# LordLiang/DrawingSpinUp

Measured on AMD Instinct MI355X. Metric: drawings/sec end-to-end (512x512, 6 views, 24 frames), higher is better.
Workload: dtype f16 (diffusion) / f16 table + f32 MLP (NSR) / f32 (stage-1 deformable convolutions, IS-Net, contour) / f32 with bf16 x 3 products (stage-2 convolutions; the reference: cuDNN TF32)

## Files before the change

### drawingspinup_amd/csrc/adamw_dev.h

```cpp
#pragma once
#include "common.h"
#include <hip/hip_fp16.h>

struct dsu_table_adamw_args {
  float4 *p, *g, *m, *v;
  __half2* img;
  int64_t n4;
  float lr, beta1, beta2, eps, wd, bc1, bc2_sqrt;
};

__device__ __forceinline__ void dsu_table_adamw_range(const dsu_table_adamw_args& a, int64_t first,
                                                      int64_t stride) {
  const float step_size = a.lr / a.bc1;
  const float omb1 = (float)(1.0 - (double)a.beta1), omb2 = (float)(1.0 - (double)a.beta2);
  for (int64_t i = first; i < a.n4; i += stride) {
    float4 P = a.p[i], G = a.g[i], M = a.m[i], V = a.v[i];
    float* pp = &P.x; float* gg = &G.x; float* mm = &M.x; float* vv = &V.x;
#pragma unroll
    for (int k = 0; k < 4; ++k) {
      float x = pp[k];
      x -= a.lr * a.wd * x;
      const float mk = mm[k] + (gg[k] - mm[k]) * omb1;
      const float vk = a.beta2 * vv[k] + omb2 * gg[k] * gg[k];
      const float denom = sqrtf(vk) / a.bc2_sqrt + a.eps;
      x -= step_size * mk / denom;
      pp[k] = x; mm[k] = mk; vv[k] = vk;
    }
    a.p[i] = P; a.m[i] = M; a.v[i] = V;
    a.g[i] = make_float4(0.0f, 0.0f, 0.0f, 0.0f);
    a.img[2 * i] = __floats2half2_rn(P.x, P.y);
    a.img[2 * i + 1] = __floats2half2_rn(P.z, P.w);
  }
}
```

### drawingspinup_amd/csrc/nsr_driver.hip

```cpp
#include "common.h"
#include "adamw_dev.h"

#include <math.h>
#include <string.h>

#include <mutex>
#include <vector>

namespace {

constexpr int N_GEO = 64 * 23 + 64 + 13 * 64 + 13;
constexpr int N_TEX = 64 * 16 + 64 + 64 * 64 + 64 + 3 * 64 + 3;
constexpr int N_SMALL = (64 * 23 + 64 + 64) + (13 * 64 + 13 + 13) + N_TEX + 1;

__device__ __forceinline__ uint4 philox(uint4 c, uint2 k) {
#pragma unroll
  for (int i = 0; i < 10; ++i) {
    const uint32_t hi0 = __umulhi(0xD2511F53u, c.x), lo0 = 0xD2511F53u * c.x;
    const uint32_t hi1 = __umulhi(0xCD9E8D57u, c.z), lo1 = 0xCD9E8D57u * c.z;
    c = make_uint4(hi1 ^ c.y ^ k.x, lo1, hi0 ^ c.w ^ k.y, lo0);
    k.x += 0x9E3779B9u;
    k.y += 0xBB67AE85u;
  }
  return c;
}
__device__ __forceinline__ float u01(uint32_t x) { return (float)(x >> 8) * (1.0f / 16777216.0f); }

__global__ __launch_bounds__(256) void nsr_draw_kernel(uint64_t seed, int64_t step, int32_t n_rays,
                                                       int32_t V, int32_t H, int32_t W,
                                                       int64_t* __restrict__ index,
                                                       int64_t* __restrict__ px,
                                                       int64_t* __restrict__ py,
                                                       float* __restrict__ jitter, int32_t n_random,
                                                       float* __restrict__ pts_random,
                                                       float* __restrict__ perturb) {
  const int i = blockIdx.x * blockDim.x + threadIdx.x;
  const uint2 key = make_uint2((uint32_t)seed, (uint32_t)(seed >> 32));
  const uint32_t s0 = (uint32_t)step, s1 = (uint32_t)((uint64_t)step >> 32);
  if (i < n_rays) {
    const uint4 r = philox(make_uint4((uint32_t)i, 0u, s0, s1), key);
    index[i] = (int64_t)(r.x % (uint32_t)V);
    px[i] = (int64_t)(r.y % (uint32_t)W);
    py[i] = (int64_t)(r.z % (uint32_t)H);
    jitter[i] = u01(r.w);
  }
  if (i < n_random) {
    const uint4 a = philox(make_uint4((uint32_t)i, 1u, s0, s1), key);
    const uint4 b = philox(make_uint4((uint32_t)i, 2u, s0, s1), key);
    pts_random[3 * i] = u01(a.x) * 2.0f - 1.0f;
    pts_random[3 * i + 1] = u01(a.y) * 2.0f - 1.0f;
    pts_random[3 * i + 2] = u01(a.z) * 2.0f - 1.0f;
    const float u1 = 1.0f - u01(b.x), u2 = u01(b.y), u3 = 1.0f - u01(b.z), u4 = u01(b.w);
    const float r1 = sqrtf(-2.0f * logf(u1)), r2 = sqrtf(-2.0f * logf(u3));
    perturb[3 * i] = r1 * cosf(6.28318530717958648f * u2);
    perturb[3 * i + 1] = r1 * sinf(6.28318530717958648f * u2);
    perturb[3 * i + 2] = r2 * cosf(6.28318530717958648f * u4);
  }
}

struct SmallArgs {
  float *w0_v, *w0_g, *b0, *w1_v, *w1_g, *b1;
  float* tex[6];
  float* variance;
  float* g_geo;
  float* g_tex;
  float* d_inv;
  float *m, *v;
  float *w0_eff, *w1_eff, *inv_s;
  float* zero_terms;
  const float* terms;
  float* terms_out;
  float lr_geo, lr_tex, lr_var, beta1, beta2, eps, wd, bc1, bc2_sqrt;
  int32_t update;
};

__device__ __forceinline__ void adamw_elem(float& x, float g, float& m, float& v, float lr,
                                           const SmallArgs& a) {
  const float omb1 = (float)(1.0 - (double)a.beta1), omb2 = (float)(1.0 - (double)a.beta2);
  x -= lr * a.wd * x;
  m = m + (g - m) * omb1;
  v = a.beta2 * v + omb2 * g * g;
  const float denom = sqrtf(v) / a.bc2_sqrt + a.eps;
  x -= (lr / a.bc1) * m / denom;
}

__global__ __launch_bounds__(1024) void small_update_kernel(SmallArgs a, dsu_table_adamw_args ta) {
  if (blockIdx.x > 0) {
    dsu_table_adamw_range(ta, (int64_t)(blockIdx.x - 1) * 1024 + threadIdx.x,
                          (int64_t)(gridDim.x - 1) * 1024);
    return;
  }
  __shared__ float s_g[N_GEO];
  __shared__ float s_v0[64 * 23], s_v1[13 * 64];
  __shared__ float s_gain[77], s_norm[77], s_dot[77];
  const int t = threadIdx.x;
  for (int i = t; i < 64 * 23; i += 1024) s_v0[i] = a.w0_v[i];
  for (int i = t; i < 13 * 64; i += 1024) s_v1[i] = a.w1_v[i];
  if (t < 77) s_gain[t] = t < 64 ? a.w0_g[t] : a.w1_g[t - 64];
  if (a.update)
    for (int i = t; i < N_GEO; i += 1024) s_g[i] = a.g_geo[i];
  __syncthreads();
  if (a.update) {
    if (t < 77) {
      const bool l0 = t < 64;
      const int r = l0 ? t : t - 64, cols = l0 ? 23 : 64;
      const float* vrow = (l0 ? s_v0 : s_v1) + r * cols;
      const float* grow = (l0 ? s_g : s_g + 64 * 23 + 64) + r * cols;
      float nn = 0.0f, dot = 0.0f;
      for (int c = 0; c < cols; ++c) {
        nn += vrow[c] * vrow[c];
        dot += grow[c] * vrow[c];
      }
      s_norm[t] = sqrtf(nn);
      s_dot[t] = dot;
    }
    __syncthreads();
    int off = 0;
    for (int i = t; i < 64 * 23; i += 1024) {
      const int r = i / 23;
      const float nrm = s_norm[r];
      const float g = (s_gain[r] / nrm) * (s_g[i] - s_v0[i] * s_dot[r] / (nrm * nrm));
      float x = s_v0[i], m = a.m[off + i], v = a.v[off + i];
      adamw_elem(x, g, m, v, a.lr_geo, a);
      a.w0_v[i] = x; a.m[off + i] = m; a.v[off + i] = v;
      s_v0[i] = x;
    }
    off += 64 * 23;
    float new_gain = 0.0f;
    if (t < 64) {
      float x = s_gain[t], m = a.m[off + t], v = a.v[off + t];
      adamw_elem(x, s_dot[t] / s_norm[t], m, v, a.lr_geo, a);
      a.w0_g[t] = x; a.m[off + t] = m; a.v[off + t] = v;
      new_gain = x;
    }
    off += 64;
    if (t < 64) {
      float x = a.b0[t], m = a.m[off + t], v = a.v[off + t];
      adamw_elem(x, s_g[64 * 23 + t], m, v, a.lr_geo, a);
      a.b0[t] = x; a.m[off + t] = m; a.v[off + t] = v;
    }
    off += 64;
    for (int i = t; i < 13 * 64; i += 1024) {
      const int r = i / 64;
      const float nrm = s_norm[64 + r];
      const float g = (s_gain[64 + r] / nrm) *
                      (s_g[64 * 23 + 64 + i] - s_v1[i] * s_dot[64 + r] / (nrm * nrm));
      float x = s_v1[i], m = a.m[off + i], v = a.v[off + i];
      adamw_elem(x, g, m, v, a.lr_geo, a);
      a.w1_v[i] = x; a.m[off + i] = m; a.v[off + i] = v;
      s_v1[i] = x;
    }
    off += 13 * 64;
    float new_gain1 = 0.0f;
    if (t < 13) {
      float x = s_gain[64 + t], m = a.m[off + t], v = a.v[off + t];
      adamw_elem(x, s_dot[64 + t] / s_norm[64 + t], m, v, a.lr_geo, a);
      a.w1_g[t] = x; a.m[off + t] = m; a.v[off + t] = v;
      new_gain1 = x;
    }
    off += 13;
    if (t < 13) {
      float x = a.b1[t], m = a.m[off + t], v = a.v[off + t];
      adamw_elem(x, s_g[64 * 23 + 64 + 13 * 64 + t], m, v, a.lr_geo, a);
      a.b1[t] = x; a.m[off + t] = m; a.v[off + t] = v;
    }
    off += 13;
    const int tn[6] = {64 * 16, 64, 64 * 64, 64, 3 * 64, 3};
    int go = 0;
    for (int k = 0; k < 6; ++k) {
      float* p = a.tex[k];
      for (int i = t; i < tn[k]; i += 1024) {
        float x = p[i], m = a.m[off + i], v = a.v[off + i];
        adamw_elem(x, a.g_tex[go + i], m, v, a.lr_tex, a);
        p[i] = x; a.m[off + i] = m; a.v[off + i] = v;
      }
      off += tn[k];
      go += tn[k];
    }
    if (t == 1023) {
      float x = a.variance[0], m = a.m[off], v = a.v[off];
      const float g = a.d_inv[0] * expf(x * 10.0f) * 10.0f;
      adamw_elem(x, g, m, v, a.lr_var, a);
      a.variance[0] = x; a.m[off] = m; a.v[off] = v;
      a.inv_s[0] = expf(x * 10.0f);
      a.d_inv[0] = 0.0f;
    }
    if (t < 3) a.zero_terms[t] = 0.0f;
    if (t >= 8 && t < 16 && a.terms_out) a.terms_out[t - 8] = a.terms[t - 8];
    __syncthreads();
    if (t < 64) s_gain[t] = new_gain;
    if (t < 13) s_gain[64 + t] = new_gain1;
    for (int i = t; i < N_GEO; i += 1024) a.g_geo[i] = 0.0f;
    for (int i = t; i < N_TEX; i += 1024) a.g_tex[i] = 0.0f;
    __syncthreads();
  } else if (t == 1023) {
    a.inv_s[0] = expf(a.variance[0] * 10.0f);
  }
  if (t < 77) {
    const bool l0 = t < 64;
    const int r = l0 ? t : t - 64, cols = l0 ? 23 : 64;
    const float* vrow = (l0 ? s_v0 : s_v1) + r * cols;
    float nn = 0.0f;
    for (int c = 0; c < cols; ++c) nn += vrow[c] * vrow[c];
    s_norm[t] = s_gain[t] / sqrtf(nn);
  }
  __syncthreads();
  for (int i = t; i < 64 * 23; i += 1024) a.w0_eff[i] = s_v0[i] * s_norm[i / 23];
  for (int i = t; i < 13 * 64; i += 1024) a.w1_eff[i] = s_v1[i] * s_norm[64 + i / 64];
}

struct Carve {
  char* base;
  int64_t off = 0;
  template <typename T>
  T* take(int64_t count) {
    off = (off + 255) / 256 * 256;
    T* p = base ? reinterpret_cast<T*>(base + off) : nullptr;
    off += count * (int64_t)sizeof(T);
    return p;
  }
};

struct Prefetch {
  int64_t *index, *px, *py;
  float *jitter, *rays, *rgb, *normal, *mask, *cosines, *vw, *tmin, *tmax;
  int32_t *counts, *offsets, *stats;
  float *rays_o, *rays_d;
  float *pts_random, *perturb;
  float *points, *t_starts, *t_ends, *sorted;
  int32_t* perm;
  void* sort_ws;
};

struct Layout {
  Prefetch pf[3];
  float *scratch_ts, *scratch_te;
  float *a_sdf, *a_grad, *a_feat;
  void* enc_cache;
  float *normal, *rgb, *alpha, *w, *comp, *d_comp, *terms;
  float *d_sdf_all, *d_grad_all, *d_feat_all, *d_normal, *d_rgb;
  void *tex_ws, *sdf_ws;
  int32_t* tex_map;
  uint32_t* tex_mask;
  float *g_geo, *g_tex, *d_inv;
  float *w0_eff, *w1_eff, *inv_s, *adam_m, *adam_v;
  int64_t tex_ws_bytes, sdf_ws_bytes, sort_ws_bytes, enc_cache_bytes, total;
};

int32_t march_row_capacity(float radius, float step) {
  const double diag = sqrt(3.0 * (2.0 * radius) * (2.0 * radius));
  return (int32_t)(diag / step) + 8;
}

int carve(const dsu_nsr_driver_cfg& c, char* base, Layout& L) {
  Carve k{base};
  const int64_t R = c.cap_rays, N = c.cap_points, nr = c.n_random, rows = N + 2 * nr;
  const int32_t rowcap = march_row_capacity(c.radius, c.render_step_size);
  L.sort_ws_bytes = c.sort_bits ? dsu_spatial_sort_workspace_bytes(rows, c.sort_bits) : 0;
  L.tex_ws_bytes = dsu_texture_bwd_workspace_bytes(N);
  L.sdf_ws_bytes = dsu_sdf_fd_bwd_workspace_bytes(&c.grid, rows);
  L.enc_cache_bytes = dsu_sdf_fd_enc_cache_bytes(rows, c.grid.n_levels);
  if (L.sort_ws_bytes < 0 || L.tex_ws_bytes < 0 || L.sdf_ws_bytes < 0 || L.enc_cache_bytes < 0)
    return DSU_EINVAL;
  for (int p = 0; p < 3; ++p) {
    Prefetch& f = L.pf[p];
    f.index = k.take<int64_t>(R); f.px = k.take<int64_t>(R); f.py = k.take<int64_t>(R);
    f.jitter = k.take<float>(R); f.rays = k.take<float>(R * 6); f.rgb = k.take<float>(R * 4);
    f.normal = k.take<float>(R * 3); f.mask = k.take<float>(R); f.cosines = k.take<float>(R);
    f.vw = k.take<float>(R); f.tmin = k.take<float>(R); f.tmax = k.take<float>(R);
    f.counts = k.take<int32_t>(R); f.offsets = k.take<int32_t>(R); f.stats = k.take<int32_t>(4);
    f.rays_o = k.take<float>(R * 3); f.rays_d = k.take<float>(R * 3);
    f.pts_random = k.take<float>(nr * 3); f.perturb = k.take<float>(nr * 3);
    f.points = k.take<float>(rows * 3); f.t_starts = k.take<float>(N); f.t_ends = k.take<float>(N);
    f.sorted = k.take<float>(rows * 3); f.perm = k.take<int32_t>(rows);
    f.sort_ws = k.take<char>(L.sort_ws_bytes > 4 ? L.sort_ws_bytes : 4);
  }
  L.scratch_ts = k.take<float>(R * (int64_t)rowcap);
  L.scratch_te = k.take<float>(R * (int64_t)rowcap);
  L.a_sdf = k.take<float>(rows); L.a_grad = k.take<float>(rows * 3); L.a_feat = k.take<float>(rows * 13);
  L.enc_cache = k.take<char>(L.enc_cache_bytes);
  L.normal = k.take<float>(N * 3); L.rgb = k.take<float>(N * 3);
  L.alpha = k.take<float>(N); L.w = k.take<float>(N);
  L.comp = k.take<float>(R * 8); L.d_comp = k.take<float>(R * 8); L.terms = k.take<float>(16);
  L.d_sdf_all = k.take<float>(rows); L.d_grad_all = k.take<float>(rows * 3);
  L.d_feat_all = k.take<float>(rows * 13);
  L.d_normal = k.take<float>(N * 3); L.d_rgb = k.take<float>(N * 3);
  L.tex_ws = k.take<char>(L.tex_ws_bytes > 4 ? L.tex_ws_bytes : 4);
  L.sdf_ws = k.take<char>(L.sdf_ws_bytes > 4 ? L.sdf_ws_bytes : 4);
  L.tex_map = k.take<int32_t>(dsu_texture_partial_map(nullptr));
  L.tex_mask = k.take<uint32_t>(N * 2);
  L.g_geo = k.take<float>(N_GEO + N_TEX + 1);
// ... 102 lines not shown
    DSU_HIP(hipMemcpy2DAsync(f.rays_d, 3 * sizeof(float), a.inj_rays + 3, 6 * sizeof(float),
                             3 * sizeof(float), n, hipMemcpyDeviceToDevice, s));
  } else {
    DSU_TRY(dsu_ortho_ray_batch_split(index, px, py, n_rays, c.c2w, c.origins, c.directions, c.images,
                                      c.image_channels, c.normals, c.masks, c.view_weights, c.H, c.W,
                                      f.rays, f.rgb, f.normal, f.mask, f.cosines, f.vw, f.rays_o,
                                      f.rays_d, s));
  }
  DSU_TRY(dsu_ray_aabb(f.rays_o, f.rays_d, n_rays, d->aabb, a.randomized ? jitter : nullptr,
                       c.render_step_size, f.tmin, f.tmax, s));
  DSU_TRY(dsu_ray_march_scratch(f.rays_o, f.rays_d, f.tmin, f.tmax, n_rays, d->aabb, a.occ_binary,
                                a.occ_binary ? a.occ_res : 0, c.render_step_size, d->rowcap,
                                f.counts, d->L.scratch_ts, d->L.scratch_te, s));
  return DSU_OK;
}

int enqueue_pack(dsu_nsr_driver* d, int p, int32_t n_rays, const dsu_nsr_step_args& a,
                 bool injected, hipStream_t s) {
  const dsu_nsr_driver_cfg& c = d->cfg;
  Prefetch& f = d->L.pf[p];
  const float* pts_random = (injected && a.inj_pts_random) ? a.inj_pts_random : f.pts_random;
  const float* perturb = (injected && a.inj_perturb) ? a.inj_perturb : f.perturb;
  DSU_TRY(dsu_ray_offsets(f.counts, n_rays, f.offsets, f.stats, s));
  DSU_TRY(dsu_ray_compact_points_cap(d->L.scratch_ts, d->L.scratch_te, d->rowcap, f.offsets,
                                     f.counts, n_rays, f.rays_o, f.rays_d, f.t_starts, f.t_ends,
                                     f.points, c.cap_points, s));
  DSU_TRY(dsu_points_tail(f.points, (int64_t)c.cap_points + 2 * c.n_random, f.stats, pts_random,
                          perturb, c.n_random, 1e-2f, s));
  if (c.sort_bits)
    DSU_TRY(dsu_spatial_sort_dev(f.points, (int64_t)c.cap_points + 2 * c.n_random, f.stats,
                                 2 * c.n_random, c.radius, c.sort_bits, f.perm, f.sorted,
                                 f.sort_ws, d->L.sort_ws_bytes, s));
  DSU_HIP(hipMemcpyAsync(d->host_stats + 2 * p, f.stats, 2 * sizeof(int32_t),
                         hipMemcpyDeviceToHost, s));
  return DSU_OK;
}

int enqueue_samples(dsu_nsr_driver* d, int p, int64_t step, int32_t n_rays,
                    const dsu_nsr_step_args& a, bool injected, hipStream_t s) {
  DSU_TRY(enqueue_march(d, p, step, n_rays, a, injected, s));
  return enqueue_pack(d, p, n_rays, a, injected, s);
}

int mark(dsu_nsr_driver* d, int family, hipStream_t s) {
  if (!d->timing) return DSU_OK;
  hipEvent_t e;
  DSU_HIP(hipEventCreate(&e));
  DSU_HIP(hipEventRecord(e, s));
  d->ev[family].push_back(e);
  return DSU_OK;
}

int launch_small_update(dsu_nsr_driver* d, const dsu_nsr_step_args* a, int update, hipStream_t s) {
  const dsu_nsr_driver_cfg& c = d->cfg;
  SmallArgs sa;
  sa.w0_v = c.w0_v; sa.w0_g = c.w0_g; sa.b0 = c.b0; sa.w1_v = c.w1_v; sa.w1_g = c.w1_g; sa.b1 = c.b1;
  for (int k = 0; k < 6; ++k) sa.tex[k] = c.tex[k];
  sa.variance = c.variance;
  sa.g_geo = d->L.g_geo; sa.g_tex = d->L.g_tex; sa.d_inv = d->L.d_inv;
  sa.m = d->L.adam_m; sa.v = d->L.adam_v;
  sa.w0_eff = d->L.w0_eff; sa.w1_eff = d->L.w1_eff; sa.inv_s = d->L.inv_s;
  sa.zero_terms = d->L.terms + 8 * (int)((a->step + 1) & 1) + 4;
  sa.terms = d->L.terms + 8 * (int)(a->step & 1);
  sa.terms_out = update ? a->terms_out : nullptr;
  sa.beta1 = c.beta1; sa.beta2 = c.beta2; sa.eps = c.adam_eps; sa.wd = c.weight_decay;
  sa.update = update;
  sa.lr_geo = sa.lr_tex = sa.lr_var = 0.0f;
  sa.bc1 = sa.bc2_sqrt = 1.0f;
  if (update) {
    sa.lr_geo = a->lr_geometry; sa.lr_tex = a->lr_texture; sa.lr_var = a->lr_variance;
    sa.bc1 = (float)(1.0 - pow((double)c.beta1, (double)a->adam_step));
    sa.bc2_sqrt = (float)sqrt(1.0 - pow((double)c.beta2, (double)a->adam_step));
  }
  dsu_table_adamw_args ta{};
  int table_blocks = 0;
  if (update && a->table_p) {
    if (a->table_n < 0 || (a->table_n & 3) || !a->table_grad || !a->table_m || !a->table_v ||
        !a->table_img || !(a->table_bc1 > 0.0f) || !(a->table_bc2_sqrt > 0.0f))
      return DSU_EINVAL;
    ta = dsu_table_adamw_args{(float4*)a->table_p, (float4*)a->table_grad, (float4*)a->table_m,
                              (float4*)a->table_v, (__half2*)const_cast<void*>(a->table_img),
                              a->table_n / 4, a->table_lr, c.beta1, c.beta2, a->table_eps,
                              a->table_wd, a->table_bc1, a->table_bc2_sqrt};
    table_blocks = (int)((ta.n4 + 1023) / 1024 < 512 ? (ta.n4 + 1023) / 1024 : 512);
  }
  small_update_kernel<<<dim3(1 + table_blocks), dim3(1024), 0, s>>>(sa, ta);
  DSU_CHECK_LAUNCH();
  return DSU_OK;
}

}

extern "C" {

int dsu_nsr_draws(uint64_t seed, int64_t step, int32_t n_rays, int32_t V, int32_t H, int32_t W,
                  int64_t* index, int64_t* x, int64_t* y, float* jitter, int32_t n_random,
                  float* pts_random, float* perturb, void* stream) {
  if (n_rays < 0 || n_random < 0 || V < 1 || H < 1 || W < 1 ||
      (n_rays && (!index || !x || !y || !jitter)) || (n_random && (!pts_random || !perturb)))
    return DSU_EINVAL;
  const int n = n_rays > n_random ? n_rays : n_random;
  if (n == 0) return DSU_OK;
  nsr_draw_kernel<<<dim3((n + 255) / 256), dim3(256), 0, (hipStream_t)stream>>>(
      seed, step, n_rays, V, H, W, index, x, y, jitter, n_random, pts_random, perturb);
  DSU_CHECK_LAUNCH();
  return DSU_OK;
}

int64_t dsu_nsr_driver_workspace_bytes(const dsu_nsr_driver_cfg* cfg) {
  if (!cfg || !cfg_ok(*cfg)) return DSU_EINVAL;
  Layout L;
  if (carve(*cfg, nullptr, L) != DSU_OK) return DSU_EINVAL;
  return L.total;
}

int dsu_nsr_driver_create(const dsu_nsr_driver_cfg* cfg, dsu_nsr_driver** out) {
  if (!cfg || !out || !cfg_ok(*cfg) || !cfg->workspace) return DSU_EINVAL;
  const void* need[] = {cfg->c2w, cfg->origins, cfg->directions, cfg->images, cfg->normals,
                        cfg->masks, cfg->view_weights, cfg->w0_v, cfg->w0_g, cfg->b0, cfg->w1_v,
                        cfg->w1_g, cfg->b1, cfg->variance, cfg->tex[0], cfg->tex[1], cfg->tex[2],
                        cfg->tex[3], cfg->tex[4], cfg->tex[5]};
  for (const void* p : need)
    if (!p) return DSU_EINVAL;
  dsu_nsr_driver* d = new dsu_nsr_driver();
  d->cfg = *cfg;
  if (carve(*cfg, (char*)cfg->workspace, d->L) != DSU_OK || d->L.total > cfg->workspace_bytes) {
    delete d;
    return DSU_EINVAL;
  }
  for (int k = 0; k < 3; ++k) {
    d->aabb[k] = -cfg->radius;
    d->aabb[3 + k] = cfg->radius;
  }
  d->rowcap = march_row_capacity(cfg->radius, cfg->render_step_size);
  {
    std::vector<int32_t> map((size_t)dsu_texture_partial_map(nullptr));
    dsu_texture_partial_map(map.data());
    if (hipMemcpy(d->L.tex_map, map.data(), map.size() * sizeof(int32_t), hipMemcpyHostToDevice) !=
        hipSuccess) {
      delete d;
      return DSU_ELAUNCH;
    }
  }
  int lo = 0, hi = 0;
  const int side_prio = dsu_nsr_side_priority_value;
  d->side_level = side_prio;
  bool ok = hipGetDevice(&d->side_device) == hipSuccess;
  if (ok && dsu_nsr_side_pool_value) d->side = side_pool_take(d->side_device, side_prio);
  ok = ok && (d->side != nullptr ||
              (hipDeviceGetStreamPriorityRange(&lo, &hi) == hipSuccess &&
               hipStreamCreateWithPriority(&d->side, hipStreamNonBlocking,
                                           side_prio == 1 ? hi : (side_prio == 2 ? 0 : lo)) == hipSuccess));
  for (int p = 0; p < 3; ++p)
    ok = ok && hipEventCreateWithFlags(&d->ready[p], hipEventDisableTiming) == hipSuccess;
  ok = ok && hipEventCreateWithFlags(&d->gate, hipEventDisableTiming) == hipSuccess &&
       hipHostMalloc((void**)&d->host_stats, 6 * sizeof(int32_t), hipHostMallocDefault) == hipSuccess;
  if (!ok) {
    dsu_nsr_driver_destroy(d);
    return DSU_ELAUNCH;
  }
  *out = d;
  return DSU_OK;
}

void dsu_nsr_driver_destroy(dsu_nsr_driver* d) {
  if (!d) return;
  if (d->side) {
    (void)hipStreamSynchronize(d->side);
    if (dsu_nsr_side_pool_value) side_pool_give(d->side_device, d->side_level, d->side);
// ... 206 lines not shown
```

### drawingspinup_amd/csrc/nsr_step.hip

```cpp
#include "common.h"
#include "adamw_dev.h"
#include <math.h>

namespace {

constexpr int RL_THREADS = 1024;

__device__ __forceinline__ uint32_t flipf(float f) {
  const uint32_t u = __float_as_uint(f);
  return (u & 0x80000000u) ? ~u : (u | 0x80000000u);
}
__device__ __forceinline__ float unflipf(uint32_t k) {
  return __uint_as_float((k & 0x80000000u) ? (k & 0x7fffffffu) : ~k);
}

__device__ __forceinline__ float wave_sum(float v) {
#pragma unroll
  for (int o = 32; o > 0; o >>= 1) v += __shfl_xor(v, o);
  return v;
}
__device__ __forceinline__ int wave_sum_i(int v) {
#pragma unroll
  for (int o = 32; o > 0; o >>= 1) v += __shfl_xor(v, o);
  return v;
// ... 306 lines not shown
                                      : (threadIdx.x == 1 ? inv_nr * lambda_sp : inv_3nr * lambda_sm);
    if (t != 0.0f) atomicAdd(&terms[threadIdx.x], t * sc);
  }
}

__global__ __launch_bounds__(1024) void ray_offsets_kernel(const int32_t* __restrict__ counts,
                                                           int64_t n, int32_t* __restrict__ offsets,
                                                           int32_t* __restrict__ stats) {
  __shared__ int red[32];
  constexpr int PER = 8;
  int carry = 0, mx = 0;
  for (int64_t base = 0; base < n; base += (int64_t)blockDim.x * PER) {
    const int64_t i0 = base + (int64_t)threadIdx.x * PER;
    int c[PER], tsum = 0;
#pragma unroll
    for (int k = 0; k < PER; ++k) {
      c[k] = i0 + k < n ? counts[i0 + k] : 0;
      mx = max(mx, c[k]);
      tsum += c[k];
    }
    int total;
    int ex = carry + block_excl_scan(tsum, red, &total);
#pragma unroll
    for (int k = 0; k < PER; ++k) {
      if (i0 + k < n) offsets[i0 + k] = ex;
      ex += c[k];
    }
    carry += total;
  }
#pragma unroll
  for (int o = 32; o > 0; o >>= 1) mx = max(mx, __shfl_xor(mx, o));
  __syncthreads();
  if ((threadIdx.x & 63) == 0) red[threadIdx.x >> 6] = mx;
  __syncthreads();
  if (threadIdx.x == 0) {
    int m = 0;
    for (int w = 0; w < (int)(blockDim.x >> 6); ++w) m = max(m, red[w]);
    stats[0] = carry;
    stats[1] = m;
  }
}

__global__ __launch_bounds__(256) void ortho_ray_batch_kernel(
    const int64_t* __restrict__ index, const int64_t* __restrict__ px, const int64_t* __restrict__ py,
    int64_t n, const float* __restrict__ c2w , const float* __restrict__ origins,
    const float* __restrict__ directions, const float* __restrict__ images, int img_c,
    const float* __restrict__ normals, const float* __restrict__ masks,
    const float* __restrict__ vweights, int H, int W, float* __restrict__ rays ,
    float* __restrict__ rgb, float* __restrict__ normal, float* __restrict__ mask,
    float* __restrict__ cosines, float* __restrict__ vw, float* __restrict__ rays_o ,
    float* __restrict__ rays_d) {
  const int64_t i = blockIdx.x * (int64_t)blockDim.x + threadIdx.x;
  if (i >= n) return;
  const int64_t v = index[i];
  const int64_t pix = (v * H + py[i]) * W + px[i];
  const float* M = c2w + v * 12;
  const float o0 = origins[pix * 3], o1 = origins[pix * 3 + 1], o2 = origins[pix * 3 + 2];
  const float d0 = directions[pix * 3], d1 = directions[pix * 3 + 1], d2 = directions[pix * 3 + 2];
  float ro[3], rd[3];
#pragma unroll
  for (int r = 0; r < 3; ++r) {
    rd[r] = (M[r * 4] * d0 + M[r * 4 + 1] * d1) + M[r * 4 + 2] * d2;
    ro[r] = M[r * 4 + 3] + ((M[r * 4] * o0 + M[r * 4 + 1] * o1) + M[r * 4 + 2] * o2);
  }
  const float nx = normals[pix * 3], ny = normals[pix * 3 + 1], nz = normals[pix * 3 + 2];
  const float dn = sqrtf((rd[0] * rd[0] + rd[1] * rd[1]) + rd[2] * rd[2]);
  const float nn = sqrtf((nx * nx + ny * ny) + nz * nz);
  const float da = fmaxf(dn, 1e-6f), na = fmaxf(nn, 1e-6f);
  cosines[i] = ((rd[0] / da) * (nx / na) + (rd[1] / da) * (ny / na)) + (rd[2] / da) * (nz / na);
  const float dz = fmaxf(dn, 1e-12f);
  rays[i * 6 + 0] = ro[0]; rays[i * 6 + 1] = ro[1]; rays[i * 6 + 2] = ro[2];
  rays[i * 6 + 3] = rd[0] / dz; rays[i * 6 + 4] = rd[1] / dz; rays[i * 6 + 5] = rd[2] / dz;
  if (rays_o) {
    rays_o[i * 3] = ro[0]; rays_o[i * 3 + 1] = ro[1]; rays_o[i * 3 + 2] = ro[2];
    rays_d[i * 3] = rd[0] / dz; rays_d[i * 3 + 1] = rd[1] / dz; rays_d[i * 3 + 2] = rd[2] / dz;
  }
  for (int c = 0; c < img_c; ++c) rgb[i * img_c + c] = images[pix * img_c + c];
  normal[i * 3] = nx; normal[i * 3 + 1] = ny; normal[i * 3 + 2] = nz;
  mask[i] = masks[pix];
  vw[i] = vweights[pix];
}


__global__ __launch_bounds__(256) void table_adamw_kernel(dsu_table_adamw_args a) {
  dsu_table_adamw_range(a, blockIdx.x * (int64_t)blockDim.x + threadIdx.x,
                        (int64_t)gridDim.x * blockDim.x);
}

struct AdamwMultiArgs {
  dsu_adamw_tensor t[DSU_ADAMW_MAX_TENSORS];
  float beta1, beta2, eps, wd;
};

__global__ __launch_bounds__(256) void adamw_multi_kernel(AdamwMultiArgs a) {
  const dsu_adamw_tensor t = a.t[blockIdx.y];
  const float step_size = t.lr / t.bias_correction1;
  const float omb1 = (float)(1.0 - (double)a.beta1), omb2 = (float)(1.0 - (double)a.beta2);
  for (int64_t i = blockIdx.x * (int64_t)blockDim.x + threadIdx.x; i < t.n;
       i += (int64_t)gridDim.x * blockDim.x) {
    const float g = t.g[i];
    float x = t.p[i];
    x -= t.lr * a.wd * x;
    const float mk = t.m[i] + (g - t.m[i]) * omb1;
    const float vk = a.beta2 * t.v[i] + omb2 * g * g;
    x -= step_size * mk / (sqrtf(vk) / t.bias_correction2_sqrt + a.eps);
    t.p[i] = x; t.m[i] = mk; t.v[i] = vk;
  }
}

__global__ __launch_bounds__(256) void table_decay_kernel(float4* __restrict__ p,
                                                          __half2* __restrict__ img, int64_t n4,
                                                          float factor) {
  for (int64_t i = blockIdx.x * (int64_t)blockDim.x + threadIdx.x; i < n4;
       i += (int64_t)gridDim.x * blockDim.x) {
    float4 P = p[i];
    P.x *= factor; P.y *= factor; P.z *= factor; P.w *= factor;
    p[i] = P;
    img[2 * i] = __floats2half2_rn(P.x, P.y);
    img[2 * i + 1] = __floats2half2_rn(P.z, P.w);
  }
}

}

extern "C" {

int dsu_table_adamw(float* p, float* g, float* m, float* v, void* img_f16, int64_t n, float lr,
                    float beta1, float beta2, float eps, float weight_decay, float bias_correction1,
                    float bias_correction2_sqrt, void* stream) {
  if (n < 0 || (n & 3) || (n && (!p || !g || !m || !v || !img_f16))) return DSU_EINVAL;
  if (!(bias_correction1 > 0.0f) || !(bias_correction2_sqrt > 0.0f)) return DSU_EINVAL;
  if (n == 0) return DSU_OK;
  table_adamw_kernel<<<dsu_capped_blocks(n / 4, 256, 2048), 256, 0, (hipStream_t)stream>>>(
      dsu_table_adamw_args{(float4*)p, (float4*)g, (float4*)m, (float4*)v, (__half2*)img_f16, n / 4,
                           lr, beta1, beta2, eps, weight_decay, bias_correction1,
                           bias_correction2_sqrt});
  DSU_CHECK_LAUNCH();
  return DSU_OK;
}

int dsu_adamw_multi(const dsu_adamw_tensor* tensors, int32_t count, float beta1, float beta2,
                    float eps, float weight_decay, void* stream) {
  if (count < 0 || count > DSU_ADAMW_MAX_TENSORS || (count && !tensors)) return DSU_EINVAL;
  if (count == 0) return DSU_OK;
  AdamwMultiArgs a;
  int64_t nmax = 0;
  for (int i = 0; i < count; ++i) {
    const dsu_adamw_tensor& t = tensors[i];
    if (t.n < 0 || (t.n && (!t.p || !t.g || !t.m || !t.v))) return DSU_EINVAL;
    if (!(t.bias_correction1 > 0.0f) || !(t.bias_correction2_sqrt > 0.0f)) return DSU_EINVAL;
    a.t[i] = t;
    if (t.n > nmax) nmax = t.n;
  }
  a.beta1 = beta1; a.beta2 = beta2; a.eps = eps; a.wd = weight_decay;
  if (nmax == 0) return DSU_OK;
  adamw_multi_kernel<<<dim3(dsu_capped_blocks(nmax, 256, 64), count), 256, 0, (hipStream_t)stream>>>(a);
  DSU_CHECK_LAUNCH();
  return DSU_OK;
}

int dsu_table_decay(float* p, void* img_f16, int64_t n, float factor, void* stream) {
  if (n < 0 || (n & 3) || (n && (!p || !img_f16))) return DSU_EINVAL;
  if (n == 0) return DSU_OK;
  table_decay_kernel<<<dsu_capped_blocks(n / 4, 256, 2048), 256, 0, (hipStream_t)stream>>>(
      (float4*)p, (__half2*)img_f16, n / 4, factor);
  DSU_CHECK_LAUNCH();
  return DSU_OK;
}

int dsu_ortho_ray_batch(const int64_t* index, const int64_t* x, const int64_t* y, int64_t n,
                        const float* c2w, const float* origins, const float* directions,
                        const float* images, int32_t image_channels, const float* normals,
                        const float* masks, const float* view_weights, int32_t H, int32_t W,
                        float* rays, float* rgb, float* normal, float* mask, float* cosines,
                        float* vw, void* stream) {
  return dsu_ortho_ray_batch_split(index, x, y, n, c2w, origins, directions, images, image_channels,
                                   normals, masks, view_weights, H, W, rays, rgb, normal, mask,
                                   cosines, vw, nullptr, nullptr, stream);
}

int dsu_ortho_ray_batch_split(const int64_t* index, const int64_t* x, const int64_t* y, int64_t n,
                              const float* c2w, const float* origins, const float* directions,
                              const float* images, int32_t image_channels, const float* normals,
                              const float* masks, const float* view_weights, int32_t H, int32_t W,
                              float* rays, float* rgb, float* normal, float* mask, float* cosines,
                              float* vw, float* rays_o, float* rays_d, void* stream) {
  if (n < 0 || H <= 0 || W <= 0 || image_channels <= 0) return DSU_EINVAL;
  if ((rays_o == nullptr) != (rays_d == nullptr)) return DSU_EINVAL;
  if (n == 0) return DSU_OK;
  if (!index || !x || !y || !c2w || !origins || !directions || !images || !normals || !masks ||
      !view_weights || !rays || !rgb || !normal || !mask || !cosines || !vw)
    return DSU_EINVAL;
  ortho_ray_batch_kernel<<<dsu_blocks_for(n, 256), 256, 0, (hipStream_t)stream>>>(
      index, x, y, n, c2w, origins, directions, images, image_channels, normals, masks, view_weights,
      H, W, rays, rgb, normal, mask, cosines, vw, rays_o, rays_d);
  DSU_CHECK_LAUNCH();
  return DSU_OK;
}

int dsu_ray_losses(const float* comp, const float* rgb, const float* normal, const float* mask,
                   const float* cosines, const float* view_weights, int32_t n_rays,
                   const dsu_ray_loss_cfg* cfg, float* terms, float* d_comp, void* stream) {
  if (!cfg || !terms || n_rays < 0) return DSU_EINVAL;
  if (n_rays && (!comp || !rgb || !normal || !mask || !cosines || !view_weights || !d_comp))
    return DSU_EINVAL;
  if (n_rays > DSU_RAY_LOSS_MAX_RAYS) return DSU_EUNSUP;
  int P = RL_THREADS;
  while (P < n_rays) P <<= 1;
  const size_t shm = (size_t)P * 16 + 256;
  DSU_ENSURE_DYN_LDS(ray_losses_kernel, shm);
  ray_losses_kernel<<<3, RL_THREADS, shm, (hipStream_t)stream>>>(
      comp, rgb, normal, mask, cosines, view_weights, n_rays, P, *cfg, terms, d_comp);
  DSU_CHECK_LAUNCH();
  return DSU_OK;
}

// ... 28 lines not shown
```

Baseline: 0.3651.

## Split small NSR optimizer update across workgroups and unroll table AdamW by two

```diff
diff --git a/drawingspinup_amd/csrc/adamw_dev.h b/drawingspinup_amd/csrc/adamw_dev.h
--- a/drawingspinup_amd/csrc/adamw_dev.h
+++ b/drawingspinup_amd/csrc/adamw_dev.h
@@ -9,26 +9,54 @@
   float lr, beta1, beta2, eps, wd, bc1, bc2_sqrt;
 };
 
+constexpr int DSU_TABLE_ADAMW_GROUPS = 2;
+constexpr int DSU_TABLE_ADAMW_THREADS = 256;
+inline int dsu_table_adamw_blocks(int64_t n4, int cap) {
+  const int64_t per = (int64_t)DSU_TABLE_ADAMW_THREADS * DSU_TABLE_ADAMW_GROUPS;
+  const int64_t b = (n4 + per - 1) / per;
+  return (int)(b < 1 ? 1 : (b > cap ? cap : b));
+}
+
+__device__ __forceinline__ void dsu_table_adamw_group(const dsu_table_adamw_args& a, float step_size,
+                                                      float omb1, float omb2, float4& P,
+                                                      const float4& G, float4& M, float4& V) {
+  float* pp = &P.x; const float* gg = &G.x; float* mm = &M.x; float* vv = &V.x;
+#pragma unroll
+  for (int k = 0; k < 4; ++k) {
+    float x = pp[k];
+    x -= a.lr * a.wd * x;
+    const float mk = mm[k] + (gg[k] - mm[k]) * omb1;
+    const float vk = a.beta2 * vv[k] + omb2 * gg[k] * gg[k];
+    const float denom = sqrtf(vk) / a.bc2_sqrt + a.eps;
+    x -= step_size * mk / denom;
+    pp[k] = x; mm[k] = mk; vv[k] = vk;
+  }
+}
+
+__device__ __forceinline__ void dsu_table_adamw_store(const dsu_table_adamw_args& a, int64_t i,
+                                                      const float4& P, const float4& M,
+                                                      const float4& V) {
+  a.p[i] = P; a.m[i] = M; a.v[i] = V;
+  a.g[i] = make_float4(0.0f, 0.0f, 0.0f, 0.0f);
+  a.img[2 * i] = __floats2half2_rn(P.x, P.y);
+  a.img[2 * i + 1] = __floats2half2_rn(P.z, P.w);
+}
+
 __device__ __forceinline__ void dsu_table_adamw_range(const dsu_table_adamw_args& a, int64_t first,
                                                       int64_t stride) {
   const float step_size = a.lr / a.bc1;
   const float omb1 = (float)(1.0 - (double)a.beta1), omb2 = (float)(1.0 - (double)a.beta2);
-  for (int64_t i = first; i < a.n4; i += stride) {
-    float4 P = a.p[i], G = a.g[i], M = a.m[i], V = a.v[i];
-    float* pp = &P.x; float* gg = &G.x; float* mm = &M.x; float* vv = &V.x;
-#pragma unroll
-    for (int k = 0; k < 4; ++k) {
-      float x = pp[k];
-      x -= a.lr * a.wd * x;
-      const float mk = mm[k] + (gg[k] - mm[k]) * omb1;
-      const float vk = a.beta2 * vv[k] + omb2 * gg[k] * gg[k];
-      const float denom = sqrtf(vk) / a.bc2_sqrt + a.eps;
-      x -= step_size * mk / denom;
-      pp[k] = x; mm[k] = mk; vv[k] = vk;
+  for (int64_t i = first; i < a.n4; i += DSU_TABLE_ADAMW_GROUPS * stride) {
+    const int64_t i1 = i + stride;
+    const bool two = i1 < a.n4;
+    float4 P0 = a.p[i], G0 = a.g[i], M0 = a.m[i], V0 = a.v[i];
+    float4 P1 = P0, G1 = G0, M1 = M0, V1 = V0;
+    if (two) { P1 = a.p[i1]; G1 = a.g[i1]; M1 = a.m[i1]; V1 = a.v[i1]; }
+    dsu_table_adamw_group(a, step_size, omb1, omb2, P0, G0, M0, V0);
+    dsu_table_adamw_store(a, i, P0, M0, V0);
+    if (two) {
+      dsu_table_adamw_group(a, step_size, omb1, omb2, P1, G1, M1, V1);
+      dsu_table_adamw_store(a, i1, P1, M1, V1);
     }
-    a.p[i] = P; a.m[i] = M; a.v[i] = V;
-    a.g[i] = make_float4(0.0f, 0.0f, 0.0f, 0.0f);
-    a.img[2 * i] = __floats2half2_rn(P.x, P.y);
-    a.img[2 * i + 1] = __floats2half2_rn(P.z, P.w);
   }
 }
diff --git a/drawingspinup_amd/csrc/nsr_driver.hip b/drawingspinup_amd/csrc/nsr_driver.hip
--- a/drawingspinup_amd/csrc/nsr_driver.hip
+++ b/drawingspinup_amd/csrc/nsr_driver.hip
@@ -84,30 +84,53 @@
   x -= (lr / a.bc1) * m / denom;
 }
 
-__global__ __launch_bounds__(1024) void small_update_kernel(SmallArgs a, dsu_table_adamw_args ta) {
-  if (blockIdx.x > 0) {
-    dsu_table_adamw_range(ta, (int64_t)(blockIdx.x - 1) * 1024 + threadIdx.x,
-                          (int64_t)(gridDim.x - 1) * 1024);
-    return;
-  }
-  __shared__ float s_g[N_GEO];
-  __shared__ float s_v0[64 * 23], s_v1[13 * 64];
-  __shared__ float s_gain[77], s_norm[77], s_dot[77];
+constexpr int SU_THREADS = DSU_TABLE_ADAMW_THREADS;
+constexpr int SU_TEX_PER_WG = 4 * SU_THREADS;
+constexpr int SU_TEX_WGS = (N_TEX + SU_TEX_PER_WG - 1) / SU_TEX_PER_WG;
+constexpr int SU_SMALL_WGS = 2 + SU_TEX_WGS;
+constexpr int M_L0 = 0, M_L1 = 64 * 23 + 64 + 64, M_TEX = M_L1 + 13 * 64 + 13 + 13, M_VAR = M_TEX + N_TEX;
+static_assert(M_VAR + 1 == N_SMALL, "moment layout: w0_v w0_g b0 w1_v w1_g b1 tex[0..5] variance");
+
+template <int ROWS, int COLS>
+__device__ __forceinline__ void su_geo_layer(float* wv, float* wg, float* b, float* gw, float* gb,
+                                             float* m, float* v, float* w_eff, const SmallArgs& a) {
+  constexpr int N = ROWS * COLS, PER = (N + SU_THREADS - 1) / SU_THREADS;
+  static_assert(ROWS <= SU_THREADS, "one thread per row");
+  __shared__ float s_v[N], s_g[N];
+  __shared__ float s_gain[ROWS], s_norm[ROWS], s_dot[ROWS];
   const int t = threadIdx.x;
-  for (int i = t; i < 64 * 23; i += 1024) s_v0[i] = a.w0_v[i];
-  for (int i = t; i < 13 * 64; i += 1024) s_v1[i] = a.w1_v[i];
-  if (t < 77) s_gain[t] = t < 64 ? a.w0_g[t] : a.w1_g[t - 64];
-  if (a.update)
-    for (int i = t; i < N_GEO; i += 1024) s_g[i] = a.g_geo[i];
+  const bool upd = a.update != 0;
+  float xv[PER], gv[PER], mv[PER], vv[PER];
+#pragma unroll
+  for (int n = 0; n < PER; ++n) {
+    const int i = t + n * SU_THREADS;
+    xv[n] = gv[n] = mv[n] = vv[n] = 0.0f;
+    if (i < N) {
+      xv[n] = wv[i];
+      if (upd) { gv[n] = gw[i]; mv[n] = m[i]; vv[n] = v[i]; }
+    }
+  }
+  float xg = 0.0f, mg = 0.0f, vg = 0.0f, xb = 0.0f, gbv = 0.0f, mb = 0.0f, vb = 0.0f;
+  if (t < ROWS) {
+    xg = wg[t];
+    if (upd) {
+      mg = m[N + t]; vg = v[N + t];
+      xb = b[t]; gbv = gb[t]; mb = m[N + ROWS + t]; vb = v[N + ROWS + t];
+    }
+  }
+#pragma unroll
+  for (int n = 0; n < PER; ++n) {
+    const int i = t + n * SU_THREADS;
+    if (i < N) { s_v[i] = xv[n]; s_g[i] = gv[n]; }
+  }
+  if (t < ROWS) s_gain[t] = xg;
   __syncthreads();
-  if (a.update) {
-    if (t < 77) {
-      const bool l0 = t < 64;
-      const int r = l0 ? t : t - 64, cols = l0 ? 23 : 64;
-      const float* vrow = (l0 ? s_v0 : s_v1) + r * cols;
-      const float* grow = (l0 ? s_g : s_g + 64 * 23 + 64) + r * cols;
+  if (upd) {
+    if (t < ROWS) {
+      const float* vrow = s_v + t * COLS;
+      const float* grow = s_g + t * COLS;
       float nn = 0.0f, dot = 0.0f;
-      for (int c = 0; c < cols; ++c) {
+      for (int c = 0; c < COLS; ++c) {
         nn += vrow[c] * vrow[c];
         dot += grow[c] * vrow[c];
       }
@@ -115,98 +138,102 @@
       s_dot[t] = dot;
     }
     __syncthreads();
-    int off = 0;
-    for (int i = t; i < 64 * 23; i += 1024) {
-      const int r = i / 23;
-      const float nrm = s_norm[r];
-      const float g = (s_gain[r] / nrm) * (s_g[i] - s_v0[i] * s_dot[r] / (nrm * nrm));
-      float x = s_v0[i], m = a.m[off + i], v = a.v[off + i];
-      adamw_elem(x, g, m, v, a.lr_geo, a);
-      a.w0_v[i] = x; a.m[off + i] = m; a.v[off + i] = v;
-      s_v0[i] = x;
-    }
-    off += 64 * 23;
-    float new_gain = 0.0f;
-    if (t < 64) {
-      float x = s_gain[t], m = a.m[off + t], v = a.v[off + t];
-      adamw_elem(x, s_dot[t] / s_norm[t], m, v, a.lr_geo, a);
-      a.w0_g[t] = x; a.m[off + t] = m; a.v[off + t] = v;
-      new_gain = x;
-    }
-    off += 64;
-    if (t < 64) {
-      float x = a.b0[t], m = a.m[off + t], v = a.v[off + t];
-      adamw_elem(x, s_g[64 * 23 + t], m, v, a.lr_geo, a);
-      a.b0[t] = x; a.m[off + t] = m; a.v[off + t] = v;
-    }
-    off += 64;
-    for (int i = t; i < 13 * 64; i += 1024) {
-      const int r = i / 64;
-      const float nrm = s_norm[64 + r];
-      const float g = (s_gain[64 + r] / nrm) *
-                      (s_g[64 * 23 + 64 + i] - s_v1[i] * s_dot[64 + r] / (nrm * nrm));
-      float x = s_v1[i], m = a.m[off + i], v = a.v[off + i];
-      adamw_elem(x, g, m, v, a.lr_geo, a);
-      a.w1_v[i] = x; a.m[off + i] = m; a.v[off + i] = v;
-      s_v1[i] = x;
-    }
-    off += 13 * 64;
-    float new_gain1 = 0.0f;
-    if (t < 13) {
-      float x = s_gain[64 + t], m = a.m[off + t], v = a.v[off + t];
-      adamw_elem(x, s_dot[64 + t] / s_norm[64 + t], m, v, a.lr_geo, a);
-      a.w1_g[t] = x; a.m[off + t] = m; a.v[off + t] = v;
-      new_gain1 = x;
-    }
-    off += 13;
-    if (t < 13) {
-      float x = a.b1[t], m = a.m[off + t], v = a.v[off + t];
-      adamw_elem(x, s_g[64 * 23 + 64 + 13 * 64 + t], m, v, a.lr_geo, a);
-      a.b1[t] = x; a.m[off + t] = m; a.v[off + t] = v;
-    }
-    off += 13;
-    const int tn[6] = {64 * 16, 64, 64 * 64, 64, 3 * 64, 3};
-    int go = 0;
-    for (int k = 0; k < 6; ++k) {
-      float* p = a.tex[k];
-      for (int i = t; i < tn[k]; i += 1024) {
-        float x = p[i], m = a.m[off + i], v = a.v[off + i];
-        adamw_elem(x, a.g_tex[go + i], m, v, a.lr_tex, a);
-        p[i] = x; a.m[off + i] = m; a.v[off + i] = v;
+#pragma unroll
+    for (int n = 0; n < PER; ++n) {
+      const int i = t + n * SU_THREADS;
+      if (i < N) {
+        const int r = i / COLS;
+        const float nrm = s_norm[r];
+        const float g = (s_gain[r] / nrm) * (gv[n] - xv[n] * s_dot[r] / (nrm * nrm));
+        adamw_elem(xv[n], g, mv[n], vv[n], a.lr_geo, a);
+        wv[i] = xv[n]; m[i] = mv[n]; v[i] = vv[n];
+        gw[i] = 0.0f;
       }
-      off += tn[k];
-      go += tn[k];
-    }
-    if (t == 1023) {
-      float x = a.variance[0], m = a.m[off], v = a.v[off];
-      const float g = a.d_inv[0] * expf(x * 10.0f) * 10.0f;
-      adamw_elem(x, g, m, v, a.lr_var, a);
-      a.variance[0] = x; a.m[off] = m; a.v[off] = v;
-      a.inv_s[0] = expf(x * 10.0f);
-      a.d_inv[0] = 0.0f;
-    }
-    if (t < 3) a.zero_terms[t] = 0.0f;
-    if (t >= 8 && t < 16 && a.terms_out) a.terms_out[t - 8] = a.terms[t - 8];
+    }
+    if (t < ROWS) {
+      adamw_elem(xg, s_dot[t] / s_norm[t], mg, vg, a.lr_geo, a);
+      wg[t] = xg; m[N + t] = mg; v[N + t] = vg;
+      adamw_elem(xb, gbv, mb, vb, a.lr_geo, a);
+      b[t] = xb; m[N + ROWS + t] = mb; v[N + ROWS + t] = vb;
+      gb[t] = 0.0f;
+    }
     __syncthreads();
-    if (t < 64) s_gain[t] = new_gain;
-    if (t < 13) s_gain[64 + t] = new_gain1;
-    for (int i = t; i < N_GEO; i += 1024) a.g_geo[i] = 0.0f;
-    for (int i = t; i < N_TEX; i += 1024) a.g_tex[i] = 0.0f;
+#pragma unroll
+    for (int n = 0; n < PER; ++n) {
+      const int i = t + n * SU_THREADS;
+      if (i < N) s_v[i] = xv[n];
+    }
+    if (t < ROWS) s_gain[t] = xg;
     __syncthreads();
-  } else if (t == 1023) {
-    a.inv_s[0] = expf(a.variance[0] * 10.0f);
-  }
-  if (t < 77) {
-    const bool l0 = t < 64;
-    const int r = l0 ? t : t - 64, cols = l0 ? 23 : 64;
-    const float* vrow = (l0 ? s_v0 : s_v1) + r * cols;
+  }
+  if (t < ROWS) {
+    const float* vrow = s_v + t * COLS;
     float nn = 0.0f;
-    for (int c = 0; c < cols; ++c) nn += vrow[c] * vrow[c];
+    for (int c = 0; c < COLS; ++c) nn += vrow[c] * vrow[c];
     s_norm[t] = s_gain[t] / sqrtf(nn);
   }
   __syncthreads();
-  for (int i = t; i < 64 * 23; i += 1024) a.w0_eff[i] = s_v0[i] * s_norm[i / 23];
-  for (int i = t; i < 13 * 64; i += 1024) a.w1_eff[i] = s_v1[i] * s_norm[64 + i / 64];
+#pragma unroll
+  for (int n = 0; n < PER; ++n) {
+    const int i = t + n * SU_THREADS;
+    if (i < N) w_eff[i] = xv[n] * s_norm[i / COLS];
+  }
+}
+
+__global__ __launch_bounds__(SU_THREADS) void small_update_kernel(SmallArgs a, dsu_table_adamw_args ta) {
+  const int t = threadIdx.x, wg = blockIdx.x;
+  if (wg >= SU_SMALL_WGS) {
+    dsu_table_adamw_range(ta, (int64_t)(wg - SU_SMALL_WGS) * SU_THREADS + t,
+                          (int64_t)(gridDim.x - SU_SMALL_WGS) * SU_THREADS);
+    return;
+  }
+  if (wg == 0) {
+    su_geo_layer<64, 23>(a.w0_v, a.w0_g, a.b0, a.g_geo, a.g_geo + 64 * 23, a.m + M_L0, a.v + M_L0,
+                         a.w0_eff, a);
+    if (a.update) {
+      if (t < 3) a.zero_terms[t] = 0.0f;
+      if (t >= 8 && t < 16 && a.terms_out) a.terms_out[t - 8] = a.terms[t - 8];
+    }
+  } else if (wg == 1) {
+    float* g1 = a.g_geo + 64 * 23 + 64;
+    su_geo_layer<13, 64>(a.w1_v, a.w1_g, a.b1, g1, g1 + 13 * 64, a.m + M_L1, a.v + M_L1, a.w1_eff, a);
+    if (t == SU_THREADS - 1) {
+      if (a.update) {
+        float x = a.variance[0], m = a.m[M_VAR], v = a.v[M_VAR];
+        const float g = a.d_inv[0] * expf(x * 10.0f) * 10.0f;
+        adamw_elem(x, g, m, v, a.lr_var, a);
+        a.variance[0] = x; a.m[M_VAR] = m; a.v[M_VAR] = v;
+        a.inv_s[0] = expf(x * 10.0f);
+        a.d_inv[0] = 0.0f;
+      } else {
+        a.inv_s[0] = expf(a.variance[0] * 10.0f);
+      }
+    }
+  } else if (a.update) {
+    constexpr int e0 = 64 * 16, e1 = e0 + 64, e2 = e1 + 64 * 64, e3 = e2 + 64, e4 = e3 + 3 * 64;
+    float* p[4];
+    float x[4], g[4], m[4], v[4];
+#pragma unroll
+    for (int n = 0; n < 4; ++n) {
+      const int j = (wg - 2) * SU_TEX_PER_WG + n * SU_THREADS + t;
+      p[n] = nullptr;
+      x[n] = g[n] = m[n] = v[n] = 0.0f;
+      if (j < N_TEX) {
+        p[n] = j < e0 ? a.tex[0] + j : j < e1 ? a.tex[1] + (j - e0) : j < e2 ? a.tex[2] + (j - e1)
+             : j < e3 ? a.tex[3] + (j - e2) : j < e4 ? a.tex[4] + (j - e3) : a.tex[5] + (j - e4);
+        x[n] = *p[n]; g[n] = a.g_tex[j]; m[n] = a.m[M_TEX + j]; v[n] = a.v[M_TEX + j];
+      }
+    }
+#pragma unroll
+    for (int n = 0; n < 4; ++n) {
+      const int j = (wg - 2) * SU_TEX_PER_WG + n * SU_THREADS + t;
+      if (j < N_TEX) {
+        adamw_elem(x[n], g[n], m[n], v[n], a.lr_tex, a);
+        *p[n] = x[n]; a.m[M_TEX + j] = m[n]; a.v[M_TEX + j] = v[n];
+        a.g_tex[j] = 0.0f;
+      }
+    }
+  }
 }
 
 struct Carve {
@@ -475,9 +502,9 @@
                               (float4*)a->table_v, (__half2*)const_cast<void*>(a->table_img),
                               a->table_n / 4, a->table_lr, c.beta1, c.beta2, a->table_eps,
                               a->table_wd, a->table_bc1, a->table_bc2_sqrt};
-    table_blocks = (int)((ta.n4 + 1023) / 1024 < 512 ? (ta.n4 + 1023) / 1024 : 512);
-  }
-  small_update_kernel<<<dim3(1 + table_blocks), dim3(1024), 0, s>>>(sa, ta);
+    if (ta.n4 > 0) table_blocks = dsu_table_adamw_blocks(ta.n4, 2048);
+  }
+  small_update_kernel<<<dim3(SU_SMALL_WGS + table_blocks), dim3(SU_THREADS), 0, s>>>(sa, ta);
   DSU_CHECK_LAUNCH();
   return DSU_OK;
 }
diff --git a/drawingspinup_amd/csrc/nsr_step.hip b/drawingspinup_amd/csrc/nsr_step.hip
--- a/drawingspinup_amd/csrc/nsr_step.hip
+++ b/drawingspinup_amd/csrc/nsr_step.hip
@@ -412,7 +412,7 @@
 }
 
 
-__global__ __launch_bounds__(256) void table_adamw_kernel(dsu_table_adamw_args a) {
+__global__ __launch_bounds__(DSU_TABLE_ADAMW_THREADS) void table_adamw_kernel(dsu_table_adamw_args a) {
   dsu_table_adamw_range(a, blockIdx.x * (int64_t)blockDim.x + threadIdx.x,
                         (int64_t)gridDim.x * blockDim.x);
 }
@@ -461,7 +461,8 @@
   if (n < 0 || (n & 3) || (n && (!p || !g || !m || !v || !img_f16))) return DSU_EINVAL;
   if (!(bias_correction1 > 0.0f) || !(bias_correction2_sqrt > 0.0f)) return DSU_EINVAL;
   if (n == 0) return DSU_OK;
-  table_adamw_kernel<<<dsu_capped_blocks(n / 4, 256, 2048), 256, 0, (hipStream_t)stream>>>(
+  table_adamw_kernel<<<dsu_table_adamw_blocks(n / 4, 2048), DSU_TABLE_ADAMW_THREADS, 0,
+                       (hipStream_t)stream>>>(
       dsu_table_adamw_args{(float4*)p, (float4*)g, (float4*)m, (float4*)v, (__half2*)img_f16, n / 4,
                            lr, beta1, beta2, eps, weight_decay, bias_correction1,
                            bias_correction2_sqrt});
```

Result: no change. 0.3619 (-0.9%).
